# kuetuofa/Transformer

Measured on AMD Instinct MI355X. Metric: tokens/sec (whole node), Transformer-base NMT training, higher is better.
Workload: dtype bf16; 1 GPU; model=transformer-base, num_layers=6, d_model=512, num_heads=8, dff=2048, global_batch=64, seq_len=256, vocab=32770, parallelism=dp1

## Files before the change

### transformer_amd/models/transformer.py

```python

from __future__ import annotations

import math

import torch
import torch.nn as nn

from .. import ops
from ..ops import reference as R


def _glorot(out_f: int, in_f: int) -> torch.Tensor:
    limit = math.sqrt(6.0 / (in_f + out_f))
    return torch.empty(out_f, in_f).uniform_(-limit, limit)


class SelfAttention(nn.Module):

    def __init__(self, d_model: int, num_heads: int):
        super().__init__()
        assert d_model % num_heads == 0
        self.d_model, self.num_heads = d_model, num_heads
        self.depth = d_model // num_heads
        w = torch.cat([_glorot(d_model, d_model) for _ in range(3)], dim=0)
        self.w_qkv = nn.Parameter(w)
        self.b_qkv = nn.Parameter(torch.zeros(3 * d_model))
        self.w_o = nn.Parameter(_glorot(d_model, d_model))
        self.b_o = nn.Parameter(torch.zeros(d_model))

    def forward(self, x, kv_pad=None, causal=False, return_weights=False):
        B, S, d = x.shape
        qkv = ops.linear(x, self.w_qkv, self.b_qkv)
        qkv = qkv.view(B, S, 3, self.num_heads, self.depth)
        out = ops.self_attention(qkv, kv_pad=kv_pad, causal=causal,
                                 return_weights=return_weights)
        if return_weights:
            out, w = out
        out = out.reshape(B, S, d)
        out = ops.linear(out, self.w_o, self.b_o)
        return (out, w) if return_weights else (out, None)


class CrossAttention(nn.Module):

    def __init__(self, d_model: int, num_heads: int):
        super().__init__()
        assert d_model % num_heads == 0
        self.d_model, self.num_heads = d_model, num_heads
        self.depth = d_model // num_heads
        self.w_q = nn.Parameter(_glorot(d_model, d_model))
        self.b_q = nn.Parameter(torch.zeros(d_model))
        w = torch.cat([_glorot(d_model, d_model) for _ in range(2)], dim=0)
        self.w_kv = nn.Parameter(w)
        self.b_kv = nn.Parameter(torch.zeros(2 * d_model))
        self.w_o = nn.Parameter(_glorot(d_model, d_model))
        self.b_o = nn.Parameter(torch.zeros(d_model))

    def forward(self, x, enc_output, kv_pad=None, return_weights=False):
        B, Sq, d = x.shape
        Sk = enc_output.shape[1]
        q = ops.linear(x, self.w_q, self.b_q).view(B, Sq, self.num_heads, self.depth)
        kv = ops.linear(enc_output, self.w_kv, self.b_kv)
        kv = kv.view(B, Sk, 2, self.num_heads, self.depth)
        out = ops.cross_attention(q, kv, kv_pad=kv_pad,
                                  return_weights=return_weights)
        if return_weights:
            out, w = out
        out = out.reshape(B, Sq, d)
        out = ops.linear(out, self.w_o, self.b_o)
        return (out, w) if return_weights else (out, None)


class FeedForward(nn.Module):

    def __init__(self, d_model: int, dff: int):
        super().__init__()
        self.w1 = nn.Parameter(_glorot(dff, d_model))
        self.b1 = nn.Parameter(torch.zeros(dff))
        self.w2 = nn.Parameter(_glorot(d_model, dff))
        self.b2 = nn.Parameter(torch.zeros(d_model))

    def forward(self, x):
        h = ops.linear(x, self.w1, self.b1, activation="relu")
        return ops.linear(h, self.w2, self.b2)


class _LN(nn.Module):
    def __init__(self, d_model: int, eps: float = 1e-6):
        super().__init__()
        self.gamma = nn.Parameter(torch.ones(d_model))
        self.beta = nn.Parameter(torch.zeros(d_model))
        self.eps = eps


class EncoderLayer(nn.Module):

    def __init__(self, d_model, num_heads, dff, rate=0.1):
        super().__init__()
        self.mha = SelfAttention(d_model, num_heads)
        self.ffn = FeedForward(d_model, dff)
        self.ln1 = _LN(d_model)
        self.ln2 = _LN(d_model)
        self.rate = rate

    def forward(self, x, kv_pad, training):
        attn, _ = self.mha(x, kv_pad=kv_pad, causal=False)
        out1 = ops.dropout_residual_layernorm(attn, x, self.ln1.gamma,
                                              self.ln1.beta, self.rate,
                                              training, self.ln1.eps)
        ffn = self.ffn(out1)
        return ops.dropout_residual_layernorm(ffn, out1, self.ln2.gamma,
                                              self.ln2.beta, self.rate,
                                              training, self.ln2.eps)


class DecoderLayer(nn.Module):

    def __init__(self, d_model, num_heads, dff, rate=0.1):
        super().__init__()
        self.mha1 = SelfAttention(d_model, num_heads)
        self.mha2 = CrossAttention(d_model, num_heads)
        self.ffn = FeedForward(d_model, dff)
        self.ln1 = _LN(d_model)
        self.ln2 = _LN(d_model)
        self.ln3 = _LN(d_model)
        self.rate = rate

    def forward(self, x, enc_output, tgt_pad, src_pad, training,
                return_weights=False):
        attn1, w1 = self.mha1(x, kv_pad=tgt_pad, causal=True,
                              return_weights=return_weights)
        out1 = ops.dropout_residual_layernorm(attn1, x, self.ln1.gamma,
                                              self.ln1.beta, self.rate,
                                              training, self.ln1.eps)
        attn2, w2 = self.mha2(out1, enc_output, kv_pad=src_pad,
                              return_weights=return_weights)
        out2 = ops.dropout_residual_layernorm(attn2, out1, self.ln2.gamma,
                                               self.ln2.beta, self.rate,
                                               training, self.ln2.eps)
        ffn = self.ffn(out2)
        out3 = ops.dropout_residual_layernorm(ffn, out2, self.ln3.gamma,
                                               self.ln3.beta, self.rate,
                                               training, self.ln3.eps)
        return out3, w1, w2


class Encoder(nn.Module):

    def __init__(self, num_layers, d_model, num_heads, dff, input_vocab_size,
                 rate=0.1, max_position=4096):
        super().__init__()
        self.d_model, self.num_layers = d_model, num_layers
        self.embedding = nn.Parameter(torch.empty(input_vocab_size, d_model)
                                      .uniform_(-0.05, 0.05))
        pe = R.positional_encoding(max_position, d_model).squeeze(0)
        self.register_buffer("pe", pe, persistent=False)
        self.layers = nn.ModuleList(
            EncoderLayer(d_model, num_heads, dff, rate) for _ in range(num_layers))
# ... 252 lines not shown
```

### transformer_amd/ops/__init__.py

```python

from __future__ import annotations

import importlib
import os

_EXT = None
_EXT_ERR: str | None = None


def _try_load():
    global _EXT, _EXT_ERR
    if _EXT is not None or _EXT_ERR is not None:
        return
    try:
        _EXT = importlib.import_module("transformer_amd.ops._tfmx_C")
    except ImportError as e:
        _EXT_ERR = str(e)


def ext():
    _try_load()
    if _EXT is None:
        raise RuntimeError(
            "transformer_amd HIP extension (_tfmx_C) is not built/loadable; "
# ... 5 lines not shown


def has_ext() -> bool:
    _try_load()
    return _EXT is not None


from . import reference
from .functional import (
    linear,
    fused_attention,
    self_attention,
    cross_attention,
    residual_layernorm,
    dropout_residual_layernorm,
    embedding_scale_pe,
    embedding_scale_pe_at,
    dropout,
    masked_cross_entropy,
    masked_accuracy,
    masked_accuracy_counts,
    argmax_lastdim,
)
```

### transformer_amd/ops/csrc/bindings.cpp

```cpp
#include <torch/extension.h>

#include <vector>

torch::Tensor gemm_nt(torch::Tensor a, torch::Tensor w, torch::Tensor bias,
                      int64_t epilogue, c10::optional<torch::Tensor> out);
torch::Tensor gemm256_nt(torch::Tensor a, torch::Tensor w, torch::Tensor bias,
                         int64_t epilogue, c10::optional<torch::Tensor> out);
torch::Tensor gemm128_nt(torch::Tensor a, torch::Tensor w, torch::Tensor bias,
                         int64_t epilogue, c10::optional<torch::Tensor> out);
torch::Tensor gemm_dw(torch::Tensor dy, torch::Tensor x,
                      c10::optional<torch::Tensor> out,
                      c10::optional<torch::Tensor> db,
                      c10::optional<torch::Tensor> cw_cached);
torch::Tensor gemm_nn(torch::Tensor a, torch::Tensor b,
                      c10::optional<torch::Tensor> out);
torch::Tensor gemm_tn(torch::Tensor a, torch::Tensor b,
                      c10::optional<torch::Tensor> out);
torch::Tensor transpose2d(torch::Tensor a);
void transpose2d_into(torch::Tensor a, torch::Tensor out);
void transpose_batch(torch::Tensor desc);
torch::Tensor colsum(torch::Tensor a, c10::optional<torch::Tensor> out);
torch::Tensor gemm_uni_nt(torch::Tensor a, torch::Tensor w,
                          c10::optional<torch::Tensor> bias, int64_t epilogue,
                          c10::optional<torch::Tensor> out);
// ... 7 lines not shown
torch::Tensor relu_bwd(torch::Tensor dy, torch::Tensor y);
std::vector<torch::Tensor> relu_bwd_db(torch::Tensor dy, torch::Tensor y,
                                       c10::optional<torch::Tensor> db_out);
torch::Tensor smoke_add(torch::Tensor a, torch::Tensor b);

std::vector<torch::Tensor> ln_fwd(torch::Tensor x, torch::Tensor res,
                                  torch::Tensor gamma, torch::Tensor beta,
                                  double eps, double p, int64_t seed,
                                  c10::optional<torch::Tensor> seed_t);
std::vector<torch::Tensor> ln_bwd(torch::Tensor dy, torch::Tensor s,
                                  torch::Tensor gamma, torch::Tensor mean,
                                  torch::Tensor rstd,
                                  c10::optional<torch::Tensor> dgamma_out,
                                  c10::optional<torch::Tensor> dbeta_out,
                                  c10::optional<torch::Tensor> mask,
                                  double p);

std::vector<torch::Tensor> attn_fwd(torch::Tensor q, torch::Tensor k,
                                    torch::Tensor v, torch::Tensor kv_pad,
                                    bool causal, double scale, int64_t trv);
std::vector<torch::Tensor> attn_bwd(torch::Tensor q, torch::Tensor k,
                                    torch::Tensor v, torch::Tensor o,
                                    torch::Tensor dout, torch::Tensor lse,
                                    torch::Tensor kv_pad, bool causal,
                                    double scale, int64_t mode);

torch::Tensor embed_pe_fwd(torch::Tensor tokens, torch::Tensor weight,
                           torch::Tensor pe);
torch::Tensor embed_pe_bwd(torch::Tensor dy, torch::Tensor tokens,
                           int64_t vocab,
                           c10::optional<torch::Tensor> out);
// ... 44 lines not shown
  m.def("gemm_nt", &gemm_nt,
        "C[M,N] = A[M,K] @ W[N,K]^T + bias (epilogue: 0=none 1=relu)",
        pybind11::arg("a"), pybind11::arg("w"), pybind11::arg("bias"),
        pybind11::arg("epilogue"), pybind11::arg("out") = pybind11::none());
  m.def("gemm_dw", &gemm_dw,
        "C[N,K] = dY[M,N]^T @ X[M,K] — deep-contraction dW via tr16 reads; "
        "optional fused bias grad db[N]",
        pybind11::arg("dy"), pybind11::arg("x"),
        pybind11::arg("out") = pybind11::none(),
        pybind11::arg("db") = pybind11::none(),
        pybind11::arg("cw") = pybind11::none());
  m.def("gemm128_nt", &gemm128_nt, "128x128 NT path, no 256 dispatch (A/B)",
        pybind11::arg("a"), pybind11::arg("w"), pybind11::arg("bias"),
        pybind11::arg("epilogue"), pybind11::arg("out") = pybind11::none());
  m.def("gemm256_nt", &gemm256_nt,
        "256x256 deep-pipelined NT GEMM (K%32==0; M/N any, edge-clamped)",
        pybind11::arg("a"), pybind11::arg("w"), pybind11::arg("bias"),
        pybind11::arg("epilogue"), pybind11::arg("out") = pybind11::none());
  m.def("gemm_nn", &gemm_nn, "C[M,N] = A[M,K] @ B[K,N] (dX)",
        pybind11::arg("a"), pybind11::arg("b"),
        pybind11::arg("out") = pybind11::none());
  m.def("gemm_tn", &gemm_tn, "C[M,N] = A[K,M]^T @ B[K,N] (dW)",
        pybind11::arg("a"), pybind11::arg("b"),
        pybind11::arg("out") = pybind11::none());
  m.def("transpose2d", &transpose2d);
  m.def("transpose2d_into", &transpose2d_into,
        "transpose a into out (out rows may be padded past a's row count)");
  m.def("transpose_batch", &transpose_batch,
        "batched 64x64-tile transposes from an int64 descriptor table");
  m.def("gemm_uni_nt", &gemm_uni_nt,
        "deep-pipelined 256-tile NT fwd GEMM (+bias/ReLU)",
        pybind11::arg("a"), pybind11::arg("w"),
        pybind11::arg("bias") = c10::nullopt, pybind11::arg("epilogue") = 0,
// ... 14 lines not shown
  m.def("relu_bwd", &relu_bwd);
  m.def("relu_bwd_db", &relu_bwd_db,
        "dz = dy*(y>0) with the bias grad db = colsum(dz) fused",
        pybind11::arg("dy"), pybind11::arg("y"),
        pybind11::arg("db") = pybind11::none());
  m.def("smoke_add", &smoke_add);
  m.def("ln_fwd", &ln_fwd, pybind11::arg("x"), pybind11::arg("res"),
        pybind11::arg("gamma"), pybind11::arg("beta"), pybind11::arg("eps"),
        pybind11::arg("p") = 0.0, pybind11::arg("seed") = 0,
        pybind11::arg("seed_t") = pybind11::none());
  m.def("ln_bwd", &ln_bwd, pybind11::arg("dy"), pybind11::arg("s"),
        pybind11::arg("gamma"), pybind11::arg("mean"), pybind11::arg("rstd"),
        pybind11::arg("dgamma_out") = pybind11::none(),
        pybind11::arg("dbeta_out") = pybind11::none(),
        pybind11::arg("mask") = pybind11::none(),
        pybind11::arg("p") = 0.0);
  m.def("attn_fwd", &attn_fwd, pybind11::arg("q"), pybind11::arg("k"),
        pybind11::arg("v"), pybind11::arg("kv_pad"), pybind11::arg("causal"),
        pybind11::arg("scale"), pybind11::arg("trv") = 1);
  m.def("attn_bwd", &attn_bwd, pybind11::arg("q"), pybind11::arg("k"),
        pybind11::arg("v"), pybind11::arg("o"), pybind11::arg("dout"),
        pybind11::arg("lse"), pybind11::arg("kv_pad"), pybind11::arg("causal"),
        pybind11::arg("scale"), pybind11::arg("mode") = 0);
  m.def("embed_pe_fwd", &embed_pe_fwd);
  m.def("embed_pe_bwd", &embed_pe_bwd, pybind11::arg("dy"),
        pybind11::arg("tokens"), pybind11::arg("vocab"),
        pybind11::arg("out") = pybind11::none());
  m.def("dropout_fwd", &dropout_fwd, pybind11::arg("x"), pybind11::arg("p"),
        pybind11::arg("seed"), pybind11::arg("seed_t") = pybind11::none());
  m.def("dropout_bwd", &dropout_bwd);
  m.def("ce_fwd", &ce_fwd);
// ... 26 lines not shown
```

### transformer_amd/ops/csrc/gemm.hip

```cpp
#include "common.h"

#include <map>

#include <torch/extension.h>
#include <ATen/hip/HIPContext.h>

typedef __bf16 bf16x8 __attribute__((ext_vector_type(8)));

#define BM 128
#define BN 128
#define BK 64
#define NTHREADS 256
#define SCR_LD 136

DEV_INLINE int lds_off(int row, int col_bytes) {
  return row * (BK * 2) + (col_bytes ^ ((row & 7) << 4));
}

template <bool ALIGNED>
DEV_INLINE void stage_tile(const short* __restrict__ g, int ldg, int nrows,
                           int ncols, short* lds) {
  const int t = threadIdx.x;
#pragma unroll
  for (int p = 0; p < 4; ++p) {
// ... 458 lines not shown
          <<<(mn + 1023) / 1024, 1024, 0, stream>>>(
              cwp, has_bias ? (const short*)bias.data_ptr() : nullptr,
              (short*)c.data_ptr(), mn, N, has_bias);
    };
    if (epilogue == 1) fin(E1{}); else fin(E0{});
  } else {
    if (epilogue == 1) dis_al(E1{}, F{}); else dis_al(E0{}, F{});
  }
  return c;
}

}

bool gemm256_viable(int M, int N, int K, int lda, int ldb);
torch::Tensor gemm256_nt(torch::Tensor a, torch::Tensor w, torch::Tensor bias,
                         int64_t epilogue, c10::optional<torch::Tensor> out);

torch::Tensor gemm_nt(torch::Tensor a, torch::Tensor w, torch::Tensor bias,
                      int64_t epilogue, c10::optional<torch::Tensor> out) {
  CHECK_BF16_2D(a);
  CHECK_BF16_2D(w);
  const int M = a.size(0), K = a.size(1), N = w.size(0);
  TORCH_CHECK(w.size(1) == K, "gemm_nt: K mismatch");
  if (gemm256_viable(M, N, K, K, K))
    return gemm256_nt(a, w, bias, epilogue, out);
  return gemm_launch<false, false>(a, w, bias, epilogue, M, N, K, K, K, out);
}

torch::Tensor gemm128_nt(torch::Tensor a, torch::Tensor w, torch::Tensor bias,
                         int64_t epilogue, c10::optional<torch::Tensor> out) {
  CHECK_BF16_2D(a);
  CHECK_BF16_2D(w);
  const int M = a.size(0), K = a.size(1), N = w.size(0);
  TORCH_CHECK(w.size(1) == K, "gemm_nt: K mismatch");
  return gemm_launch<false, false>(a, w, bias, epilogue, M, N, K, K, K, out);
}

torch::Tensor gemm_nn(torch::Tensor a, torch::Tensor b,
                      c10::optional<torch::Tensor> out) {
  CHECK_BF16_2D(a);
// ... 133 lines not shown
```

### transformer_amd/ops/csrc/gemm256.hip

```cpp
#include "common.h"

#include <torch/extension.h>
#include <ATen/hip/HIPContext.h>

typedef __bf16 bf16x8g __attribute__((ext_vector_type(8)));

namespace {

#define G_BM 256
#define G_BK 64
#define G_THREADS 512
#define G_TILE_ELEMS (G_BM * G_BK)

DEV_INLINE int sw256(int off) { return off ^ (((off >> 9) & 1) << 5); }

template <int ROWS = 256>
DEV_INLINE void stage256(const short* __restrict__ g, long ldg, int row0,
                         int maxrow, int h, short* lds) {
  const int wid = threadIdx.x >> 6, lane = threadIdx.x & 63;
#pragma unroll
  for (int p = 0; p < ROWS / 128; ++p) {
    const int chunk = h * (ROWS / 16) + p * 8 + wid;
    const int d = chunk * 1024 + lane * 16;
    const int lg = sw256(d);
// ... 9 lines not shown

DEV_INLINE bf16x8g frag256(const short* lds, int row, int kb ) {
  const int off = sw256(row * 128 + kb);
  return (bf16x8g)*(const s16x8*)((const char*)lds + off);
}

#define G_BARRIER() __builtin_amdgcn_s_barrier()
#define G_WAIT_LGKM0() asm volatile("s_waitcnt lgkmcnt(0)" ::: "memory")
#define G_WAIT_VM0() asm volatile("s_waitcnt vmcnt(0)" ::: "memory")

template <int EPILOGUE, int BM_, int BN_, int ORDER = 0, int XCDMAP = 1>
__global__ __launch_bounds__(G_THREADS, 1)
void gemm256_kernel(const short* __restrict__ A, const short* __restrict__ B,
                    const short* __restrict__ bias, short* __restrict__ C,
                    int M, int N, int K, int lda, int ldb, int has_bias,
                    int nbm, int nbn) {
  constexpr int MF = BM_ / 32;
  constexpr int NF = BN_ / 64;
  constexpr int A_ELEMS = BM_ * G_BK;
  constexpr int B_ELEMS = BN_ * G_BK;
  constexpr int SLOT = A_ELEMS + B_ELEMS;
  extern __shared__ short smem[];
  const int lane = threadIdx.x & 63;

  int nwg = nbm * nbn;
  int wg = blockIdx.x;
  if (XCDMAP) {
    int q = nwg / 8, r = nwg % 8, x = wg % 8, o = wg / 8;
    wg = (x < r ? x * (q + 1) : r * (q + 1) + (x - r) * q) + o;
  }
  const int bm0 = (ORDER ? (wg % nbm) : (wg / nbn)) * BM_;
// ... 90 lines not shown

#pragma unroll
  for (int i = 0; i < MF; ++i) {
    const int grow_base = bm0 + wm + i * 16 + kg * 4;
#pragma unroll
    for (int j = 0; j < NF; ++j) {
      const int gcol = bn0 + wn + j * 16 + fr;
      if (gcol >= N) continue;
      const float bv = (has_bias && bias) ? bfbits2f(bias[gcol]) : 0.0f;
#pragma unroll
      for (int r = 0; r < 4; ++r) {
        const int grow = grow_base + r;
        if (grow >= M) continue;
        float v = acc[i][j][r] + bv;
        if (EPILOGUE == 1) v = fmaxf(v, 0.0f);
        C[(long)grow * N + gcol] = f2bfbits(v);
      }
    }
  }
}

}

static void gemm256_tile(int M, int N, int& BM, int& BN) {
  const long g22 = (long)cdiv(M, 256) * cdiv(N, 256);
  const long g21 = (long)cdiv(M, 256) * cdiv(N, 128);
  auto util = [](long nwg) {
    return nwg < 1 ? 0.0 : (double)nwg / ((nwg + 255) / 256 * 256);
  };
  if (g22 >= 224) {
    BM = 256;
// ... 1 lines not shown
  }
  else if (g21 >= 224) { BM = 256; BN = 128; }
  else { BM = 128; BN = 128; }
}

bool gemm256_viable(int M, int N, int K, int lda, int ldb) {
  if (K % G_BK != 0 || K < 2 * G_BK) return false;
  if (lda % 8 != 0 || ldb % 8 != 0) return false;
  int BM, BN;
  gemm256_tile(M, N, BM, BN);
  long nwg = (long)cdiv(M, BM) * cdiv(N, BN);
  return nwg >= 224 && (K >= 512 || nwg >= 384);
}

torch::Tensor gemm256_nt(torch::Tensor a, torch::Tensor w, torch::Tensor bias,
                         int64_t epilogue, c10::optional<torch::Tensor> out) {
  TORCH_CHECK(a.is_cuda() && a.dtype() == torch::kBFloat16 && a.dim() == 2 &&
              a.is_contiguous(), "gemm256_nt: a must be contiguous bf16 2-D");
  TORCH_CHECK(w.is_cuda() && w.dtype() == torch::kBFloat16 && w.dim() == 2 &&
              w.is_contiguous(), "gemm256_nt: w must be contiguous bf16 2-D");
  const int M = a.size(0), K = a.size(1), N = w.size(0);
  TORCH_CHECK(w.size(1) == K, "gemm256_nt: K mismatch");
  TORCH_CHECK(K % G_BK == 0 && K >= 2 * G_BK,
              "gemm256_nt: K must be a multiple of 64 (>=128)");
  const bool has_bias = bias.defined() && bias.numel() > 0;
  torch::Tensor c;
  if (out.has_value()) {
    c = *out;
    TORCH_CHECK(c.is_cuda() && c.dtype() == torch::kBFloat16 &&
                c.is_contiguous() && c.numel() == (long)M * N,
                "out must be contiguous bf16 with M*N elements");
  } else {
    c = torch::empty({M, N}, a.options());
  }
  int BMv, BNv;
  gemm256_tile(M, N, BMv, BNv);
  const int nbm = cdiv(M, BMv), nbn = cdiv(N, BNv);
  const size_t smem = 2 * ((size_t)BMv + BNv) * G_BK * sizeof(short);
  auto stream = at::hip::getCurrentHIPStream();
  static bool attr_set[2][3] = {};
  static const int env_order = [] {
    const char* e = getenv("TFMX_G256_ORDER");
    return e ? (e[0] == 'n' ? 1 : 0) : -1;
  }();
  static const int env_xcd = [] {
    const char* e = getenv("TFMX_G256_XCD");
    return e ? atoi(e) : -1;
  }();
  const int order = env_order >= 0 ? env_order : 0;
  const int xcd = env_xcd >= 0 ? env_xcd : 1;
  auto launch = [&](auto epi, auto bmc, auto bnc) {
    constexpr int E = decltype(epi)::value;
    constexpr int BM_ = decltype(bmc)::value;
    constexpr int BN_ = decltype(bnc)::value;
    constexpr int ti = BM_ == 128 ? 2 : (BN_ == 128 ? 1 : 0);
    auto go = [&](auto oc, auto xc) {
      constexpr int OV = decltype(oc)::value;
      constexpr int XV = decltype(xc)::value;
      if (!attr_set[E][ti]) {
        (void)hipFuncSetAttribute(
            (const void*)gemm256_kernel<E, BM_, BN_, OV, XV>,
            hipFuncAttributeMaxDynamicSharedMemorySize, (int)smem);
        attr_set[E][ti] = true;
      }
      gemm256_kernel<E, BM_, BN_, OV, XV>
          <<<nbm * nbn, G_THREADS, smem, stream>>>(
              (const short*)a.data_ptr(), (const short*)w.data_ptr(),
              has_bias ? (const short*)bias.data_ptr() : nullptr,
              (short*)c.data_ptr(), M, N, K, K, K, has_bias, nbm, nbn);
    };
    using I0 = std::integral_constant<int, 0>;
    using I1 = std::integral_constant<int, 1>;
    if (order) { if (xcd) go(I1{}, I1{}); else go(I1{}, I0{}); }
    else       { if (xcd) go(I0{}, I1{}); else go(I0{}, I0{}); }
  };
  using E0 = std::integral_constant<int, 0>;
  using E1 = std::integral_constant<int, 1>;
  using T256 = std::integral_constant<int, 256>;
  using T128 = std::integral_constant<int, 128>;
  auto dis = [&](auto epi) {
    if (BMv == 128) launch(epi, T128{}, T128{});
    else if (BNv == 128) launch(epi, T256{}, T128{});
    else launch(epi, T256{}, T256{});
  };
  if (epilogue == 1) dis(E1{}); else dis(E0{});
  return c;
}
```

### transformer_amd/ops/csrc/layernorm.hip

```cpp
#include "common.h"

#include <map>

#include <torch/extension.h>
#include <ATen/hip/HIPContext.h>

DEV_INLINE unsigned int ln_pcg(unsigned long long key) {
  key = key * 6364136223846793005ull + 1442695040888963407ull;
  unsigned int h = (unsigned int)((key ^ (key >> 33)) >> 11);
  h ^= h >> 16; h *= 0x7feb352dU; h ^= h >> 15; h *= 0x846ca68bU;
  h ^= h >> 16;
  return h;
}

template <bool DROP>
__global__ __launch_bounds__(256)
void ln_fwd_kernel(const short* __restrict__ x, const short* __restrict__ res,
                   const short* __restrict__ gamma,
                   const short* __restrict__ beta, short* __restrict__ y,
                   short* __restrict__ s, float* __restrict__ mean_out,
                   float* __restrict__ rstd_out, int R, int D, float eps,
                   unsigned char* __restrict__ mask, float p, float inv_keep,
                   unsigned long long seed,
                   const long long* __restrict__ seed_ptr) {
// ... 200 lines not shown
      atomicAdd(&acc_g[cc], sg);
      atomicAdd(&acc_b[cc], sb);
    }
  }
  }
  if (last_arriver((unsigned*)(acc_b + D), gridDim.x * gridDim.y)) {
    for (int i = threadIdx.x; i < D; i += 64) {
      dgamma[i] = f2bfbits(acc_g[i]);
      dbeta[i] = f2bfbits(acc_b[i]);
      acc_g[i] = 0.f;
      acc_b[i] = 0.f;
    }
    if (threadIdx.x == 0)
      __hip_atomic_store((unsigned*)(acc_b + D), 0u, __ATOMIC_RELAXED,
                         __HIP_MEMORY_SCOPE_AGENT);
  }
}

std::vector<torch::Tensor> ln_fwd(torch::Tensor x, torch::Tensor res,
                                  torch::Tensor gamma, torch::Tensor beta,
                                  double eps, double p, int64_t seed,
                                  c10::optional<torch::Tensor> seed_t) {
  TORCH_CHECK(x.is_cuda() && x.dtype() == torch::kBFloat16 && x.dim() == 2 &&
              x.is_contiguous() && res.is_contiguous());
  const int R = x.size(0), D = x.size(1);
  auto y = torch::empty_like(x);
  auto s = torch::empty_like(x);
  auto mean = torch::empty({R}, x.options().dtype(torch::kFloat32));
  auto rstd = torch::empty({R}, x.options().dtype(torch::kFloat32));
  auto stream = at::hip::getCurrentHIPStream();
// ... 7 lines not shown
        (short*)y.data_ptr(), (short*)s.data_ptr(), mean.data_ptr<float>(),
        rstd.data_ptr<float>(), R, D, (float)eps,
        mask.data_ptr<unsigned char>(), (float)p,
        1.0f / (1.0f - (float)p), (unsigned long long)seed, sp);
    return {y, s, mean, rstd, mask};
  }
  ln_fwd_kernel<false><<<cdiv(R, 4), 256, 0, stream>>>(
      (const short*)x.data_ptr(), (const short*)res.data_ptr(),
      (const short*)gamma.data_ptr(), (const short*)beta.data_ptr(),
      (short*)y.data_ptr(), (short*)s.data_ptr(), mean.data_ptr<float>(),
      rstd.data_ptr<float>(), R, D, (float)eps, nullptr, 0.f, 1.f, 0,
      nullptr);
  return {y, s, mean, rstd};
}

std::vector<torch::Tensor> ln_bwd(torch::Tensor dy, torch::Tensor s,
                                  torch::Tensor gamma, torch::Tensor mean,
                                  torch::Tensor rstd,
                                  c10::optional<torch::Tensor> dgamma_out,
                                  c10::optional<torch::Tensor> dbeta_out,
                                  c10::optional<torch::Tensor> mask,
                                  double p) {
  const int R = dy.size(0), D = dy.size(1);
  auto dx = torch::empty_like(dy);
  auto dest = [&](c10::optional<torch::Tensor>& o) {
    if (o.has_value()) {
      TORCH_CHECK(o->is_cuda() && o->dtype() == torch::kBFloat16 &&
                  o->is_contiguous() && o->numel() == D);
      return *o;
    }
    return torch::empty({D}, dy.options());
  };
  auto dgamma = dest(dgamma_out);
  auto dbeta = dest(dbeta_out);
  auto stream = at::hip::getCurrentHIPStream();
  torch::Tensor dxm;
  if (mask.has_value()) {
    dxm = torch::empty_like(dy);
    ln_bwd_kernel<true><<<cdiv(R, 4), 256, 0, stream>>>(
        (const short*)dy.data_ptr(), (const short*)s.data_ptr(),
        (const short*)gamma.data_ptr(), mean.data_ptr<float>(),
        rstd.data_ptr<float>(), (short*)dx.data_ptr(), R, D,
        mask->data_ptr<unsigned char>(), (short*)dxm.data_ptr(),
        1.0f / (1.0f - (float)p));
  } else {
    ln_bwd_kernel<false><<<cdiv(R, 4), 256, 0, stream>>>(
        (const short*)dy.data_ptr(), (const short*)s.data_ptr(),
        (const short*)gamma.data_ptr(), mean.data_ptr<float>(),
        rstd.data_ptr<float>(), (short*)dx.data_ptr(), R, D, nullptr,
        nullptr, 1.f);
  }
  static std::map<std::pair<int, int>, torch::Tensor> ws_cache;
  auto wkey = std::make_pair((int)dy.get_device(), D);
  auto wit = ws_cache.find(wkey);
  if (wit == ws_cache.end())
    wit = ws_cache.emplace(wkey, torch::zeros(
        {2L * D + 1}, dy.options().dtype(torch::kFloat32))).first;
  auto acc_g = wit->second.narrow(0, 0, D);
  auto acc_b = wit->second.narrow(0, D, D + 1);
  dim3 gbgrid(cdiv(cdiv(D, 2), 64), cdiv(R, LNGB_ROWS));
  ln_gb_kernel<<<gbgrid, 64, 0, stream>>>(
      (const short*)dy.data_ptr(), (const short*)s.data_ptr(),
      mean.data_ptr<float>(), rstd.data_ptr<float>(),
      acc_g.data_ptr<float>(), acc_b.data_ptr<float>(),
      (short*)dgamma.data_ptr(), (short*)dbeta.data_ptr(), R, D);
  if (mask.has_value()) return {dx, dgamma, dbeta, dxm};
  return {dx, dgamma, dbeta};
}
```

### transformer_amd/ops/functional.py

```python

from __future__ import annotations

import math

import os

import torch

from . import reference as R
from . import ext



def set_grad_ready_callback(params, fn):
    for p in params:
        if fn is None:
            if hasattr(p, "_grad_ready_cb"):
                del p._grad_ready_cb
        else:
            p._grad_ready_cb = fn


def _grad_ready(*params):
    for p in params:
# ... 401 lines not shown


class _DropResidualLNFlatFn(torch.autograd.Function):
    @staticmethod
    def forward(ctx, x, res, gb, p, eps):
        y = _DropResidualLNFn.forward(ctx, x, res, gb[0], gb[1], p, eps)
        ctx.flat_gb = gb
        return y

    @staticmethod
    def backward(ctx, dy):
        dxm, dres, _, _, _, _ = _DropResidualLNFn.backward(ctx, dy)
        return dxm, dres, None, None, None


def residual_layernorm(x, res, gamma, beta, eps: float = 1e-6):
    if x.is_cuda:
        shp = x.shape
        d = shp[-1]
        x2 = x.reshape(-1, d).contiguous()
        r2 = res.reshape(-1, d).contiguous()
        if _flat(gamma) is not None:
            y = _ResidualLNFlatFn.apply(x2, r2, [gamma, beta], eps)
        else:
            y = _ResidualLNFn.apply(x2, r2, gamma, beta, eps)
        return y.view(shp)
    if x.dtype in (torch.bfloat16, torch.float16):
        return R.residual_layernorm(x.float(), res.float(), gamma.float(),
                                    beta.float(), eps).to(x.dtype)
    return R.residual_layernorm(x, res, gamma, beta, eps)
# ... 174 lines not shown
```

Measured before the change: 1.772 million tokens/s.

## Fuse output projection and FFN with dropout-residual-layernorm in custom autograd

Adds autograd functions that fold the attention output projection and the whole FFN together with dropout-residual-LayerNorm, so their backward passes run as one fused sequence. The new LN backward kernel also computes the bias gradient, which removes a separate colsum pass and per-op autograd overhead. GEMM256 gains relu-mask and residual-add epilogues to fuse the FFN dx path, but these only run when TFMX_FFN_BWD=fused is set. The change adds complexity and risks gradient-plumbing errors in the flat-parameter path.

```diff
diff --git a/transformer_amd/models/transformer.py b/transformer_amd/models/transformer.py
--- a/transformer_amd/models/transformer.py
+++ b/transformer_amd/models/transformer.py
@@ -28,7 +28,8 @@
         self.w_o = nn.Parameter(_glorot(d_model, d_model))
         self.b_o = nn.Parameter(torch.zeros(d_model))
 
-    def forward(self, x, kv_pad=None, causal=False, return_weights=False):
+    def forward(self, x, kv_pad=None, causal=False, return_weights=False,
+                project=True):
         B, S, d = x.shape
         qkv = ops.linear(x, self.w_qkv, self.b_qkv)
         qkv = qkv.view(B, S, 3, self.num_heads, self.depth)
@@ -37,7 +38,8 @@
         if return_weights:
             out, w = out
         out = out.reshape(B, S, d)
-        out = ops.linear(out, self.w_o, self.b_o)
+        if project:
+            out = ops.linear(out, self.w_o, self.b_o)
         return (out, w) if return_weights else (out, None)
 
 
@@ -56,7 +58,8 @@
         self.w_o = nn.Parameter(_glorot(d_model, d_model))
         self.b_o = nn.Parameter(torch.zeros(d_model))
 
-    def forward(self, x, enc_output, kv_pad=None, return_weights=False):
+    def forward(self, x, enc_output, kv_pad=None, return_weights=False,
+                project=True):
         B, Sq, d = x.shape
         Sk = enc_output.shape[1]
         q = ops.linear(x, self.w_q, self.b_q).view(B, Sq, self.num_heads, self.depth)
@@ -67,7 +70,8 @@
         if return_weights:
             out, w = out
         out = out.reshape(B, Sq, d)
-        out = ops.linear(out, self.w_o, self.b_o)
+        if project:
+            out = ops.linear(out, self.w_o, self.b_o)
         return (out, w) if return_weights else (out, None)
 
 
@@ -83,6 +87,18 @@
     def forward(self, x):
         h = ops.linear(x, self.w1, self.b1, activation="relu")
         return ops.linear(h, self.w2, self.b2)
+
+
+def _proj_ln(mha, heads, res, ln, rate, training):
+    return ops.linear_dropout_residual_layernorm(
+        heads, mha.w_o, mha.b_o, res, ln.gamma, ln.beta, rate, training,
+        ln.eps)
+
+
+def _ffn_ln(ffn, x, ln, rate, training):
+    return ops.ffn_dropout_residual_layernorm(
+        x, ffn.w1, ffn.b1, ffn.w2, ffn.b2, ln.gamma, ln.beta, rate, training,
+        ln.eps)
 
 
 class _LN(nn.Module):
@@ -104,14 +120,9 @@
         self.rate = rate
 
     def forward(self, x, kv_pad, training):
-        attn, _ = self.mha(x, kv_pad=kv_pad, causal=False)
-        out1 = ops.dropout_residual_layernorm(attn, x, self.ln1.gamma,
-                                              self.ln1.beta, self.rate,
-                                              training, self.ln1.eps)
-        ffn = self.ffn(out1)
-        return ops.dropout_residual_layernorm(ffn, out1, self.ln2.gamma,
-                                              self.ln2.beta, self.rate,
-                                              training, self.ln2.eps)
+        heads, _ = self.mha(x, kv_pad=kv_pad, causal=False, project=False)
+        out1 = _proj_ln(self.mha, heads, x, self.ln1, self.rate, training)
+        return _ffn_ln(self.ffn, out1, self.ln2, self.rate, training)
 
 
 class DecoderLayer(nn.Module):
@@ -128,20 +139,14 @@
 
     def forward(self, x, enc_output, tgt_pad, src_pad, training,
                 return_weights=False):
-        attn1, w1 = self.mha1(x, kv_pad=tgt_pad, causal=True,
-                              return_weights=return_weights)
-        out1 = ops.dropout_residual_layernorm(attn1, x, self.ln1.gamma,
-                                              self.ln1.beta, self.rate,
-                                              training, self.ln1.eps)
-        attn2, w2 = self.mha2(out1, enc_output, kv_pad=src_pad,
-                              return_weights=return_weights)
-        out2 = ops.dropout_residual_layernorm(attn2, out1, self.ln2.gamma,
-                                               self.ln2.beta, self.rate,
-                                               training, self.ln2.eps)
-        ffn = self.ffn(out2)
-        out3 = ops.dropout_residual_layernorm(ffn, out2, self.ln3.gamma,
-                                               self.ln3.beta, self.rate,
-                                               training, self.ln3.eps)
+        heads1, w1 = self.mha1(x, kv_pad=tgt_pad, causal=True,
+                               return_weights=return_weights, project=False)
+        out1 = _proj_ln(self.mha1, heads1, x, self.ln1, self.rate, training)
+        heads2, w2 = self.mha2(out1, enc_output, kv_pad=src_pad,
+                               return_weights=return_weights, project=False)
+        out2 = _proj_ln(self.mha2, heads2, out1, self.ln2, self.rate,
+                        training)
+        out3 = _ffn_ln(self.ffn, out2, self.ln3, self.rate, training)
         return out3, w1, w2
 
 
diff --git a/transformer_amd/ops/__init__.py b/transformer_amd/ops/__init__.py
--- a/transformer_amd/ops/__init__.py
+++ b/transformer_amd/ops/__init__.py
@@ -43,6 +43,8 @@
     cross_attention,
     residual_layernorm,
     dropout_residual_layernorm,
+    linear_dropout_residual_layernorm,
+    ffn_dropout_residual_layernorm,
     embedding_scale_pe,
     embedding_scale_pe_at,
     dropout,
diff --git a/transformer_amd/ops/csrc/bindings.cpp b/transformer_amd/ops/csrc/bindings.cpp
--- a/transformer_amd/ops/csrc/bindings.cpp
+++ b/transformer_amd/ops/csrc/bindings.cpp
@@ -5,7 +5,9 @@
 torch::Tensor gemm_nt(torch::Tensor a, torch::Tensor w, torch::Tensor bias,
                       int64_t epilogue, c10::optional<torch::Tensor> out);
 torch::Tensor gemm256_nt(torch::Tensor a, torch::Tensor w, torch::Tensor bias,
-                         int64_t epilogue, c10::optional<torch::Tensor> out);
+                         int64_t epilogue, c10::optional<torch::Tensor> out,
+                         c10::optional<torch::Tensor> aux);
+bool gemm256_viable(int M, int N, int K, int lda, int ldb);
 torch::Tensor gemm128_nt(torch::Tensor a, torch::Tensor w, torch::Tensor bias,
                          int64_t epilogue, c10::optional<torch::Tensor> out);
 torch::Tensor gemm_dw(torch::Tensor dy, torch::Tensor x,
@@ -45,7 +47,8 @@
                                   c10::optional<torch::Tensor> dgamma_out,
                                   c10::optional<torch::Tensor> dbeta_out,
                                   c10::optional<torch::Tensor> mask,
-                                  double p);
+                                  double p,
+                                  c10::optional<torch::Tensor> dbias_out);
 
 std::vector<torch::Tensor> attn_fwd(torch::Tensor q, torch::Tensor k,
                                     torch::Tensor v, torch::Tensor kv_pad,
@@ -120,9 +123,15 @@
         pybind11::arg("a"), pybind11::arg("w"), pybind11::arg("bias"),
         pybind11::arg("epilogue"), pybind11::arg("out") = pybind11::none());
   m.def("gemm256_nt", &gemm256_nt,
-        "256x256 deep-pipelined NT GEMM (K%32==0; M/N any, edge-clamped)",
+        "256x256 deep-pipelined NT GEMM (K%64==0; M/N any, edge-clamped); "
+        "epilogue 0=none 1=relu, with aux (M,N): 2=relu-mask (aux>0 ? c : 0) "
+        "3=residual-add (c + aux, one rounding)",
         pybind11::arg("a"), pybind11::arg("w"), pybind11::arg("bias"),
-        pybind11::arg("epilogue"), pybind11::arg("out") = pybind11::none());
+        pybind11::arg("epilogue"), pybind11::arg("out") = pybind11::none(),
+        pybind11::arg("aux") = pybind11::none());
+  m.def("gemm256_viable",
+        [](int M, int N, int K) { return gemm256_viable(M, N, K, K, K); },
+        "whether gemm_nt dispatches (M,N,K) to the 256-tile kernel");
   m.def("gemm_nn", &gemm_nn, "C[M,N] = A[M,K] @ B[K,N] (dX)",
         pybind11::arg("a"), pybind11::arg("b"),
         pybind11::arg("out") = pybind11::none());
@@ -167,7 +176,8 @@
         pybind11::arg("dgamma_out") = pybind11::none(),
         pybind11::arg("dbeta_out") = pybind11::none(),
         pybind11::arg("mask") = pybind11::none(),
-        pybind11::arg("p") = 0.0);
+        pybind11::arg("p") = 0.0,
+        pybind11::arg("dbias_out") = pybind11::none());
   m.def("attn_fwd", &attn_fwd, pybind11::arg("q"), pybind11::arg("k"),
         pybind11::arg("v"), pybind11::arg("kv_pad"), pybind11::arg("causal"),
         pybind11::arg("scale"), pybind11::arg("trv") = 1);
diff --git a/transformer_amd/ops/csrc/gemm.hip b/transformer_amd/ops/csrc/gemm.hip
--- a/transformer_amd/ops/csrc/gemm.hip
+++ b/transformer_amd/ops/csrc/gemm.hip
@@ -496,7 +496,8 @@
 
 bool gemm256_viable(int M, int N, int K, int lda, int ldb);
 torch::Tensor gemm256_nt(torch::Tensor a, torch::Tensor w, torch::Tensor bias,
-                         int64_t epilogue, c10::optional<torch::Tensor> out);
+                         int64_t epilogue, c10::optional<torch::Tensor> out,
+                         c10::optional<torch::Tensor> aux);
 
 torch::Tensor gemm_nt(torch::Tensor a, torch::Tensor w, torch::Tensor bias,
                       int64_t epilogue, c10::optional<torch::Tensor> out) {
@@ -505,7 +506,7 @@
   const int M = a.size(0), K = a.size(1), N = w.size(0);
   TORCH_CHECK(w.size(1) == K, "gemm_nt: K mismatch");
   if (gemm256_viable(M, N, K, K, K))
-    return gemm256_nt(a, w, bias, epilogue, out);
+    return gemm256_nt(a, w, bias, epilogue, out, c10::nullopt);
   return gemm_launch<false, false>(a, w, bias, epilogue, M, N, K, K, K, out);
 }
 
diff --git a/transformer_amd/ops/csrc/gemm256.hip b/transformer_amd/ops/csrc/gemm256.hip
--- a/transformer_amd/ops/csrc/gemm256.hip
+++ b/transformer_amd/ops/csrc/gemm256.hip
@@ -47,7 +47,7 @@
 void gemm256_kernel(const short* __restrict__ A, const short* __restrict__ B,
                     const short* __restrict__ bias, short* __restrict__ C,
                     int M, int N, int K, int lda, int ldb, int has_bias,
-                    int nbm, int nbn) {
+                    int nbm, int nbn, const short* __restrict__ aux) {
   constexpr int MF = BM_ / 32;
   constexpr int NF = BN_ / 64;
   constexpr int A_ELEMS = BM_ * G_BK;
@@ -168,7 +168,11 @@
         if (grow >= M) continue;
         float v = acc[i][j][r] + bv;
         if (EPILOGUE == 1) v = fmaxf(v, 0.0f);
-        C[(long)grow * N + gcol] = f2bfbits(v);
+        if (EPILOGUE == 3) v += bfbits2f(aux[(long)grow * N + gcol]);
+        short o = f2bfbits(v);
+        if (EPILOGUE == 2)
+          o = bfbits2f(aux[(long)grow * N + gcol]) > 0.f ? o : (short)0;
+        C[(long)grow * N + gcol] = o;
       }
     }
   }
@@ -200,7 +204,8 @@
 }
 
 torch::Tensor gemm256_nt(torch::Tensor a, torch::Tensor w, torch::Tensor bias,
-                         int64_t epilogue, c10::optional<torch::Tensor> out) {
+                         int64_t epilogue, c10::optional<torch::Tensor> out,
+                         c10::optional<torch::Tensor> aux) {
   TORCH_CHECK(a.is_cuda() && a.dtype() == torch::kBFloat16 && a.dim() == 2 &&
               a.is_contiguous(), "gemm256_nt: a must be contiguous bf16 2-D");
   TORCH_CHECK(w.is_cuda() && w.dtype() == torch::kBFloat16 && w.dim() == 2 &&
@@ -209,13 +214,27 @@
   TORCH_CHECK(w.size(1) == K, "gemm256_nt: K mismatch");
   TORCH_CHECK(K % G_BK == 0 && K >= 2 * G_BK,
               "gemm256_nt: K must be a multiple of 64 (>=128)");
-  const bool has_bias = bias.defined() && bias.numel() > 0;
+  TORCH_CHECK(epilogue >= 0 && epilogue <= 3, "gemm256_nt: bad epilogue");
+  const bool has_bias = epilogue < 2 && bias.defined() && bias.numel() > 0;
+  const short* auxp = nullptr;
+  if (epilogue >= 2) {
+    TORCH_CHECK(aux.has_value() && aux->is_cuda() &&
+                aux->dtype() == torch::kBFloat16 && aux->dim() == 2 &&
+                aux->is_contiguous() && aux->size(0) == M &&
+                aux->size(1) == N,
+                "gemm256_nt: epilogue 2/3 needs a contiguous bf16 (M, N) aux");
+    TORCH_CHECK(!(bias.defined() && bias.numel() > 0),
+                "gemm256_nt: epilogue 2/3 takes no bias");
+    auxp = (const short*)aux->data_ptr();
+  }
   torch::Tensor c;
   if (out.has_value()) {
     c = *out;
     TORCH_CHECK(c.is_cuda() && c.dtype() == torch::kBFloat16 &&
                 c.is_contiguous() && c.numel() == (long)M * N,
                 "out must be contiguous bf16 with M*N elements");
+    TORCH_CHECK(!auxp || c.data_ptr() != (void*)auxp,
+                "gemm256_nt: out must not alias aux");
   } else {
     c = torch::empty({M, N}, a.options());
   }
@@ -224,7 +243,7 @@
   const int nbm = cdiv(M, BMv), nbn = cdiv(N, BNv);
   const size_t smem = 2 * ((size_t)BMv + BNv) * G_BK * sizeof(short);
   auto stream = at::hip::getCurrentHIPStream();
-  static bool attr_set[2][3] = {};
+  static bool attr_set[4][3] = {};
   static const int env_order = [] {
     const char* e = getenv("TFMX_G256_ORDER");
     return e ? (e[0] == 'n' ? 1 : 0) : -1;
@@ -253,7 +272,8 @@
           <<<nbm * nbn, G_THREADS, smem, stream>>>(
               (const short*)a.data_ptr(), (const short*)w.data_ptr(),
               has_bias ? (const short*)bias.data_ptr() : nullptr,
-              (short*)c.data_ptr(), M, N, K, K, K, has_bias, nbm, nbn);
+              (short*)c.data_ptr(), M, N, K, K, K, has_bias, nbm, nbn,
+              auxp);
     };
     using I0 = std::integral_constant<int, 0>;
     using I1 = std::integral_constant<int, 1>;
@@ -262,6 +282,8 @@
   };
   using E0 = std::integral_constant<int, 0>;
   using E1 = std::integral_constant<int, 1>;
+  using E2 = std::integral_constant<int, 2>;
+  using E3 = std::integral_constant<int, 3>;
   using T256 = std::integral_constant<int, 256>;
   using T128 = std::integral_constant<int, 128>;
   auto dis = [&](auto epi) {
@@ -269,6 +291,9 @@
     else if (BNv == 128) launch(epi, T256{}, T128{});
     else launch(epi, T256{}, T256{});
   };
-  if (epilogue == 1) dis(E1{}); else dis(E0{});
+  if (epilogue == 3) dis(E3{});
+  else if (epilogue == 2) dis(E2{});
+  else if (epilogue == 1) dis(E1{});
+  else dis(E0{});
   return c;
 }
diff --git a/transformer_amd/ops/csrc/layernorm.hip b/transformer_amd/ops/csrc/layernorm.hip
--- a/transformer_amd/ops/csrc/layernorm.hip
+++ b/transformer_amd/ops/csrc/layernorm.hip
@@ -1,5 +1,8 @@
 #include "common.h"
 
+#include <algorithm>
+#include <cstdlib>
+#include <cstring>
 #include <map>
 
 #include <torch/extension.h>
@@ -238,6 +241,180 @@
     if (threadIdx.x == 0)
       __hip_atomic_store((unsigned*)(acc_b + D), 0u, __ATOMIC_RELAXED,
                          __HIP_MEMORY_SCOPE_AGENT);
+  }
+}
+
+#define LNF_ROWS_PER_PASS 4096
+template <bool DROP, int NCH, int NW>
+__global__ __launch_bounds__(NW * 64)
+void ln_bwd_fused_kernel(const short* __restrict__ dy,
+                         const short* __restrict__ s,
+                         const short* __restrict__ gamma,
+                         const float* __restrict__ mean,
+                         const float* __restrict__ rstd,
+                         short* __restrict__ dx, int R, int D,
+                         const unsigned char* __restrict__ mask,
+                         short* __restrict__ dxm, float inv_keep,
+                         float* __restrict__ ws, short* __restrict__ dgamma,
+                         short* __restrict__ dbeta,
+                         short* __restrict__ dbias) {
+  constexpr int NQ = DROP ? 3 : 2;
+  constexpr int LW = NCH * 576;
+  constexpr int SL = NQ * LW;
+  __shared__ float red[(NW / 2) * SL];
+  const int lane = threadIdx.x & 63;
+  const int wave = threadIdx.x >> 6;
+
+  float gam[NCH][8], ag[NCH][8], ab[NCH][8], am[NCH][8];
+  bool act[NCH];
+#pragma unroll
+  for (int k = 0; k < NCH; ++k) {
+    const int c = lane * 8 + k * (WAVE * 8);
+    act[k] = c < D;
+    s16x8 gv = {0, 0, 0, 0, 0, 0, 0, 0};
+    if (act[k]) gv = *(const s16x8*)(gamma + c);
+#pragma unroll
+    for (int j = 0; j < 8; ++j) {
+      gam[k][j] = bfbits2f(gv[j]);
+      ag[k][j] = 0.f;
+      ab[k][j] = 0.f;
+      am[k][j] = 0.f;
+    }
+  }
+
+  s16x8 dv[NCH], sv[NCH], dvn[NCH], svn[NCH];
+  unsigned long long mk[NCH], mkn[NCH];
+  float mu = 0.f, rs = 0.f, mun = 0.f, rsn = 0.f;
+  auto load_row = [&](int row, s16x8 (&d)[NCH], s16x8 (&x)[NCH],
+                      unsigned long long (&m)[NCH], float& mu_, float& rs_) {
+    const long base = (long)row * D;
+    mu_ = mean[row];
+    rs_ = rstd[row];
+#pragma unroll
+    for (int k = 0; k < NCH; ++k) {
+      const int c = lane * 8 + k * (WAVE * 8);
+      d[k] = s16x8{0, 0, 0, 0, 0, 0, 0, 0};
+      x[k] = d[k];
+      m[k] = 0;
+      if (act[k]) {
+        d[k] = *(const s16x8*)(dy + base + c);
+        x[k] = *(const s16x8*)(s + base + c);
+        if (DROP) m[k] = *(const unsigned long long*)(mask + base + c);
+      }
+    }
+  };
+  const int row0 = blockIdx.x * NW + wave, rstep = gridDim.x * NW;
+  if (row0 < R) load_row(row0, dvn, svn, mkn, mun, rsn);
+  for (int row = row0; row < R; row += rstep) {
+    const long base = (long)row * D;
+    mu = mun;
+    rs = rsn;
+#pragma unroll
+    for (int k = 0; k < NCH; ++k) {
+      dv[k] = dvn[k];
+      sv[k] = svn[k];
+      mk[k] = mkn[k];
+    }
+    if (row + rstep < R) load_row(row + rstep, dvn, svn, mkn, mun, rsn);
+    float sg = 0.f, sgx = 0.f;
+    {
+#pragma clang fp contract(off)
+#pragma unroll
+      for (int k = 0; k < NCH; ++k) {
+        if (act[k]) {
+#pragma unroll
+          for (int j = 0; j < 8; ++j) {
+            float xh = (bfbits2f(sv[k][j]) - mu) * rs;
+            float g = bfbits2f(dv[k][j]) * gam[k][j];
+            float gx = g * xh;
+            sg += g;
+            sgx += gx;
+          }
+        }
+      }
+    }
+    sg = wave_sum(sg) / D;
+    sgx = wave_sum(sgx) / D;
+#pragma unroll
+    for (int k = 0; k < NCH; ++k) {
+      if (act[k]) {
+        const int c = lane * 8 + k * (WAVE * 8);
+        s16x8 xo, mo;
+#pragma unroll
+        for (int j = 0; j < 8; ++j) {
+          float xh = (bfbits2f(sv[k][j]) - mu) * rs;
+          float dyv = bfbits2f(dv[k][j]);
+          float d = rs * __builtin_fmaf(-xh, sgx,
+                                        __builtin_fmaf(dyv, gam[k][j], -sg));
+          xo[j] = f2bfbits(d);
+          ag[k][j] = __builtin_fmaf(dyv, xh, ag[k][j]);
+          ab[k][j] += dyv;
+          if (DROP) {
+            mo[j] = ((mk[k] >> (8 * j)) & 0xff) ? f2bfbits(d * inv_keep)
+                                                : (short)0;
+            am[k][j] += bfbits2f(mo[j]);
+          }
+        }
+        *(s16x8*)(dx + base + c) = xo;
+        if (DROP) *(s16x8*)(dxm + base + c) = mo;
+      }
+    }
+  }
+
+  auto park = [&](float* dst) {
+#pragma unroll
+    for (int k = 0; k < NCH; ++k) {
+      if (act[k]) {
+        const int li = (lane * 8 + k * (WAVE * 8)) / 8 * 9;
+#pragma unroll
+        for (int j = 0; j < 8; ++j) {
+          dst[li + j] = ag[k][j];
+          dst[LW + li + j] = ab[k][j];
+          if (DROP) dst[2 * LW + li + j] = am[k][j];
+        }
+      }
+    }
+  };
+#pragma unroll
+  for (int half = NW / 2; half >= 1; half >>= 1) {
+    if (wave >= half && wave < 2 * half) park(red + (wave - half) * SL);
+    __syncthreads();
+    if (wave < half) {
+      const float* src = red + wave * SL;
+#pragma unroll
+      for (int k = 0; k < NCH; ++k) {
+        if (act[k]) {
+          const int li = (lane * 8 + k * (WAVE * 8)) / 8 * 9;
+#pragma unroll
+          for (int j = 0; j < 8; ++j) {
+            ag[k][j] += src[li + j];
+            ab[k][j] += src[LW + li + j];
+            if (DROP) am[k][j] += src[2 * LW + li + j];
+          }
+        }
+      }
+    }
+    __syncthreads();
+  }
+  if (wave == 0) park(red);
+  __syncthreads();
+  const int nflush = ((DROP && dbias) ? 3 : 2) * D;
+  const int rot = (int)((blockIdx.x * 64u) % (unsigned)nflush);
+  for (int i = threadIdx.x; i < nflush; i += NW * 64) {
+    int ii = i + rot;
+    if (ii >= nflush) ii -= nflush;
+    const int q = ii / D, c = ii - q * D;
+    atomicAdd(&ws[ii], red[q * LW + c + (c >> 3)]);
+  }
+  unsigned* cnt = (unsigned*)(ws + 3 * D);
+  if (last_arriver(cnt, gridDim.x)) {
+    for (int i = threadIdx.x; i < nflush; i += NW * 64) {
+      const int q = i / D, c = i - q * D;
+      (q == 0 ? dgamma : q == 1 ? dbeta : dbias)[c] = f2bfbits(ws[i]);
+      ws[i] = 0.f;
+    }
+    if (threadIdx.x == 0)
+      __hip_atomic_store(cnt, 0u, __ATOMIC_RELAXED, __HIP_MEMORY_SCOPE_AGENT);
   }
 }
 
@@ -275,14 +452,23 @@
   return {y, s, mean, rstd};
 }
 
+torch::Tensor colsum(torch::Tensor a, c10::optional<torch::Tensor> out);
+
 std::vector<torch::Tensor> ln_bwd(torch::Tensor dy, torch::Tensor s,
                                   torch::Tensor gamma, torch::Tensor mean,
                                   torch::Tensor rstd,
                                   c10::optional<torch::Tensor> dgamma_out,
                                   c10::optional<torch::Tensor> dbeta_out,
                                   c10::optional<torch::Tensor> mask,
-                                  double p) {
+                                  double p,
+                                  c10::optional<torch::Tensor> dbias_out) {
+  TORCH_CHECK(dy.is_cuda() && dy.dtype() == torch::kBFloat16 &&
+              dy.dim() == 2 && dy.is_contiguous() && s.is_contiguous() &&
+              s.sizes() == dy.sizes(), "ln_bwd: bad dy/s");
   const int R = dy.size(0), D = dy.size(1);
+  TORCH_CHECK(mean.numel() == R && rstd.numel() == R && gamma.numel() == D &&
+              (!mask.has_value() || mask->numel() == (long)R * D),
+              "ln_bwd: shape mismatch");
   auto dx = torch::empty_like(dy);
   auto dest = [&](c10::optional<torch::Tensor>& o) {
     if (o.has_value()) {
@@ -295,9 +481,55 @@
   auto dgamma = dest(dgamma_out);
   auto dbeta = dest(dbeta_out);
   auto stream = at::hip::getCurrentHIPStream();
-  torch::Tensor dxm;
-  if (mask.has_value()) {
-    dxm = torch::empty_like(dy);
+  const bool drop = mask.has_value();
+  torch::Tensor dxm, dbias;
+  if (drop) dxm = torch::empty_like(dy);
+  if (drop && dbias_out.has_value()) dbias = dest(dbias_out);
+  static std::map<std::pair<int, int>, torch::Tensor> ws_cache;
+  auto wkey = std::make_pair((int)dy.get_device(), D);
+  auto wit = ws_cache.find(wkey);
+  if (wit == ws_cache.end())
+    wit = ws_cache.emplace(wkey, torch::zeros(
+        {3L * D + 1}, dy.options().dtype(torch::kFloat32))).first;
+  const char* arm = getenv("TFMX_LN_BWD");
+  const bool split = arm && strcmp(arm, "split") == 0;
+  if (!split && D % 8 == 0 && D <= 1024 && R > 0) {
+    const char* wv = getenv("TFMX_LN_BWD_WAVES");
+    const bool w8 = wv && atoi(wv) == 8;
+    auto launch = [&](auto dropc, auto nchc, auto nwc) {
+      constexpr bool DR = decltype(dropc)::value;
+      constexpr int NCH = decltype(nchc)::value;
+      constexpr int NW = decltype(nwc)::value;
+      const int grid = std::min(LNF_ROWS_PER_PASS / NW, cdiv(R, NW));
+      ln_bwd_fused_kernel<DR, NCH, NW><<<grid, NW * 64, 0, stream>>>(
+          (const short*)dy.data_ptr(), (const short*)s.data_ptr(),
+          (const short*)gamma.data_ptr(), mean.data_ptr<float>(),
+          rstd.data_ptr<float>(), (short*)dx.data_ptr(), R, D,
+          DR ? mask->data_ptr<unsigned char>() : nullptr,
+          DR ? (short*)dxm.data_ptr() : nullptr,
+          DR ? 1.0f / (1.0f - (float)p) : 1.f,
+          wit->second.data_ptr<float>(), (short*)dgamma.data_ptr(),
+          (short*)dbeta.data_ptr(),
+          dbias.defined() ? (short*)dbias.data_ptr() : nullptr);
+    };
+    using T = std::true_type;
+    using F = std::false_type;
+    using C1 = std::integral_constant<int, 1>;
+    using C2 = std::integral_constant<int, 2>;
+    using W8 = std::integral_constant<int, 8>;
+    using W16 = std::integral_constant<int, 16>;
+    auto by_w = [&](auto dropc, auto nchc) {
+      if (w8) launch(dropc, nchc, W8{}); else launch(dropc, nchc, W16{});
+    };
+    auto by_ch = [&](auto dropc) {
+      if (D <= 512) by_w(dropc, C1{}); else launch(dropc, C2{}, W8{});
+    };
+    if (drop) by_ch(T{}); else by_ch(F{});
+    if (dbias.defined()) return {dx, dgamma, dbeta, dxm, dbias};
+    if (drop) return {dx, dgamma, dbeta, dxm};
+    return {dx, dgamma, dbeta};
+  }
+  if (drop) {
     ln_bwd_kernel<true><<<cdiv(R, 4), 256, 0, stream>>>(
         (const short*)dy.data_ptr(), (const short*)s.data_ptr(),
         (const short*)gamma.data_ptr(), mean.data_ptr<float>(),
@@ -311,12 +543,6 @@
         rstd.data_ptr<float>(), (short*)dx.data_ptr(), R, D, nullptr,
         nullptr, 1.f);
   }
-  static std::map<std::pair<int, int>, torch::Tensor> ws_cache;
-  auto wkey = std::make_pair((int)dy.get_device(), D);
-  auto wit = ws_cache.find(wkey);
-  if (wit == ws_cache.end())
-    wit = ws_cache.emplace(wkey, torch::zeros(
-        {2L * D + 1}, dy.options().dtype(torch::kFloat32))).first;
   auto acc_g = wit->second.narrow(0, 0, D);
   auto acc_b = wit->second.narrow(0, D, D + 1);
   dim3 gbgrid(cdiv(cdiv(D, 2), 64), cdiv(R, LNGB_ROWS));
@@ -325,6 +551,7 @@
       mean.data_ptr<float>(), rstd.data_ptr<float>(),
       acc_g.data_ptr<float>(), acc_b.data_ptr<float>(),
       (short*)dgamma.data_ptr(), (short*)dbeta.data_ptr(), R, D);
-  if (mask.has_value()) return {dx, dgamma, dbeta, dxm};
+  if (dbias.defined()) return {dx, dgamma, dbeta, dxm, colsum(dxm, dbias)};
+  if (drop) return {dx, dgamma, dbeta, dxm};
   return {dx, dgamma, dbeta};
 }
diff --git a/transformer_amd/ops/functional.py b/transformer_amd/ops/functional.py
--- a/transformer_amd/ops/functional.py
+++ b/transformer_amd/ops/functional.py
@@ -439,6 +439,174 @@
         return dxm, dres, None, None, None
 
 
+
+def _ln_drop_fwd(E, a, res, gamma, beta, eps, p):
+    if _GRAPH_SEED_T is not None:
+        _GRAPH_SALT[0] += 1
+        return E.ln_fwd(a, res, gamma, beta, eps, p, _GRAPH_SALT[0],
+                        _GRAPH_SEED_T)
+    seed = int(torch.randint(0, 2**31 - 1, (1,)).item())
+    return E.ln_fwd(a, res, gamma, beta, eps, p, seed)
+
+
+def _grad_dst(p, flat):
+    if p is None:
+        return None
+    return _flat(p).view(-1) if flat else torch.empty_like(p)
+
+
+def _ln_drop_bwd(E, ctx, dy, s, gamma, mean, rstd, mask, g, bt, b):
+    flat = ctx.flat
+    dg, dbt, db = _grad_dst(g, flat), _grad_dst(bt, flat), _grad_dst(b, flat)
+    out = E.ln_bwd(dy.contiguous(), s, gamma, mean, rstd, dg, dbt, mask,
+                   ctx.p, db)
+    if flat:
+        _grad_ready(g, bt)
+    return out[0], out[3], dg, dbt, db
+
+
+class _LinearDropLNFn(torch.autograd.Function):
+
+    @staticmethod
+    def forward(ctx, x, res, w, b, gamma, beta, p, eps):
+        E = ext()
+        a = _fwd_gemm(E, x, w, b, None)
+        y, s, mean, rstd, mask = _ln_drop_fwd(E, a, res, gamma, beta, eps, p)
+        ctx.p = p
+        ctx.flat = False
+        ctx.params = (w, b, gamma, beta)
+        ctx.save_for_backward(x, s, mean, rstd, mask)
+        return y
+
+    @staticmethod
+    def backward(ctx, dy):
+        E = ext()
+        x, s, mean, rstd, mask = ctx.saved_tensors
+        w, b, g, bt = ctx.params
+        dres, dxm, dg, dbt, db = _ln_drop_bwd(E, ctx, dy, s, g, mean, rstd,
+                                              mask, g, bt, b)
+        dx = _dx_gemm(E, dxm, w)
+        if ctx.flat:
+            _dw_gemm(dxm, x, out=_flat(w).view(w.shape[0], -1))
+            _grad_ready(w, b)
+            return dx, dres, None, None, None
+        dw = _dw_gemm(dxm, x)
+        return dx, dres, dw, db, dg, dbt, None, None
+
+
+class _LinearDropLNFlatFn(torch.autograd.Function):
+
+    @staticmethod
+    def forward(ctx, x, res, params, p, eps):
+        y = _LinearDropLNFn.forward(ctx, x, res, *params, p, eps)
+        ctx.flat = True
+        return y
+
+    backward = staticmethod(_LinearDropLNFn.backward)
+
+
+def _dx_epilogue_ok(E, M, n_out, k):
+    return (os.environ.get("TFMX_FFN_BWD", "split") == "fused"
+            and _DX_BACKEND == "wt" and M >= 2048
+            and n_out % 64 == 0 and k % 64 == 0
+            and E.gemm256_viable(M, n_out, k))
+
+
+class _FFNDropLNFn(torch.autograd.Function):
+
+    @staticmethod
+    def forward(ctx, x, w1, b1, w2, b2, gamma, beta, p, eps):
+        E = ext()
+        h = _fwd_gemm(E, x, w1, b1, "relu")
+        a = _fwd_gemm(E, h, w2, b2, None)
+        y, s, mean, rstd, mask = _ln_drop_fwd(E, a, x, gamma, beta, eps, p)
+        ctx.p = p
+        ctx.flat = False
+        ctx.params = (w1, b1, w2, b2, gamma, beta)
+        ctx.save_for_backward(x, h, s, mean, rstd, mask)
+        return y
+
+    @staticmethod
+    def backward(ctx, dy):
+        E = ext()
+        x, h, s, mean, rstd, mask = ctx.saved_tensors
+        w1, b1, w2, b2, g, bt = ctx.params
+        flat = ctx.flat
+        dres, dxm, dg, dbt, db2 = _ln_drop_bwd(E, ctx, dy, s, g, mean, rstd,
+                                               mask, g, bt, b2)
+        dw2 = _dw_gemm(dxm, h, out=_flat(w2).view(w2.shape[0], -1)
+                       if flat else None)
+        if flat:
+            _grad_ready(w2, b2)
+        M, d, dff = x.shape[0], x.shape[1], h.shape[1]
+        nob = torch.Tensor()
+        if _dx_epilogue_ok(E, M, dff, d):
+            dz = E.gemm256_nt(dxm, _wt_padded(E, w2), nob, 2, None, h)
+        else:
+            dz = E.relu_bwd(_dx_gemm(E, dxm, w2).contiguous(), h)
+        dw1 = _dw_gemm(dz, x, out=_flat(w1).view(w1.shape[0], -1)
+                       if flat else None)
+        db1 = E.colsum(dz, _grad_dst(b1, flat)) if b1 is not None else None
+        if flat:
+            _grad_ready(w1, b1)
+        if _dx_epilogue_ok(E, M, d, dff):
+            dx = E.gemm256_nt(dz, _wt_padded(E, w1), nob, 3, None, dres)
+        else:
+            dx = _dx_gemm(E, dz, w1) + dres
+        if flat:
+            return dx, None, None, None
+        return dx, dw1, db1, dw2, db2, dg, dbt, None, None
+
+
+class _FFNDropLNFlatFn(torch.autograd.Function):
+    @staticmethod
+    def forward(ctx, x, params, p, eps):
+        y = _FFNDropLNFn.forward(ctx, x, *params, p, eps)
+        ctx.flat = True
+        return y
+
+    backward = staticmethod(_FFNDropLNFn.backward)
+
+
+def _all_flat(*params):
+    fl = [_flat(p) is not None for p in params if p is not None]
+    return all(fl), any(fl)
+
+
+def linear_dropout_residual_layernorm(x, w, b, res, gamma, beta, rate: float,
+                                      training: bool, eps: float = 1e-6):
+    allf, anyf = _all_flat(w, b, gamma, beta)
+    if not (x.is_cuda and training and rate > 0.0 and allf == anyf):
+        return dropout_residual_layernorm(linear(x, w, b), res, gamma, beta,
+                                          rate, training, eps)
+    shp = res.shape
+    x2 = x.reshape(-1, x.shape[-1]).contiguous()
+    r2 = res.reshape(-1, shp[-1]).contiguous()
+    if allf:
+        y = _LinearDropLNFlatFn.apply(x2, r2, [w, b, gamma, beta], rate, eps)
+    else:
+        y = _LinearDropLNFn.apply(x2, r2, w, b, gamma, beta, rate, eps)
+    return y.view(shp)
+
+
+def ffn_dropout_residual_layernorm(x, w1, b1, w2, b2, gamma, beta,
+                                   rate: float, training: bool,
+                                   eps: float = 1e-6):
+    allf, anyf = _all_flat(w1, b1, w2, b2, gamma, beta)
+    if not (x.is_cuda and training and rate > 0.0 and allf == anyf):
+        h = linear(x, w1, b1, activation="relu")
+        return dropout_residual_layernorm(linear(h, w2, b2), x, gamma, beta,
+                                          rate, training, eps)
+    shp = x.shape
+    x2 = x.reshape(-1, shp[-1]).contiguous()
+    if allf:
+        y = _FFNDropLNFlatFn.apply(x2, [w1, b1, w2, b2, gamma, beta], rate,
+                                   eps)
+    else:
+        y = _FFNDropLNFn.apply(x2, w1, b1, w2, b2, gamma, beta, rate, eps)
+    return y.view(shp)
+
+
 def residual_layernorm(x, res, gamma, beta, eps: float = 1e-6):
     if x.is_cuda:
         shp = x.shape
```

Result: faster. 1.849 million tokens/s (median of 6 runs) (+4.4%).
